# HBioquant/DiffBindFR

Measured on AMD Instinct MI355X. Metric: poses_per_sec, higher is better.
Workload: dtype f32

## Files before the change

### diffbindfr_amd/csrc/conv.hip

```cpp
#include <cstdio>
#include <cstdlib>
#include <type_traits>
#include <vector>

#include "common.h"

#ifndef CONV_PRIO
#define CONV_PRIO 0
#endif
#ifndef CONV_XPF
#define CONV_XPF 0
#endif
#ifndef CONV_NB2_WAVES
#define CONV_NB2_WAVES 2
#endif
#define XS_LD (MAXD + 4)

typedef float f32x4 __attribute__((ext_vector_type(4)));

#define TRACE_BLOCKS 1024
#define TRACE_TILES 48
#define TRACE_REC (2 + 3 * TRACE_TILES + 8)
#define RSTAMP(k) do { if ((ABL & 16) && a.trace && bid < TRACE_BLOCKS && lane == 0) a.trace[((size_t)bid * 4 + wave) * TRACE_REC + 2 + 3 * TRACE_TILES + (k)] = __builtin_amdgcn_s_memrealtime(); } while (0)
#define TSTAMP(k) do { if ((ABL & 16) && a.trace && bid < TRACE_BLOCKS && lane == 0) a.trace[((size_t)bid * 4 + wave) * TRACE_REC + 2 + 3 * TRACE_TILES + (k)] = __builtin_readcyclecounter(); } while (0)
// ... 290 lines not shown
          }
        }
#if CONV_PRIO == 1
        __builtin_amdgcn_s_setprio(0);
#elif CONV_PRIO == 2
        __builtin_amdgcn_s_setprio(3);
#endif
        if ((ABL & 16) && trc && trc_n < TRACE_TILES) {
#pragma unroll
          for (int b = 0; b < NB; ++b) asm volatile("" : "+v"(oacc[b][0]));
          if (lane == 0) trc[4 + 3 * trc_n] = __builtin_readcyclecounter();
          ++trc_n;
        }
      }
      if (flags & 2) {
#pragma unroll
        for (int b = 0; b < NB; ++b) {
          float* op = un + (16 * b + n) * O_LD + oo;
          op[0] = oacc[b][0];
          if (VOUT) { op[1] = oacc[b][1]; op[2] = oacc[b][2]; }
        }
      }
    };
    switch (type) {
      case PT_SS: run(std::integral_constant<int, PT_SS>{}); break;
      case PT_SV: run(std::integral_constant<int, PT_SV>{}); break;
      case PT_VS: run(std::integral_constant<int, PT_VS>{}); break;
      case PT_VVS: run(std::integral_constant<int, PT_VVS>{}); break;
      case PT_VVV: run(std::integral_constant<int, PT_VVV>{}); break;
      default: run(std::integral_constant<int, PT_VTV>{}); break;
    }
  }
  TSTAMP(3);
  RSTAMP(7);
  __syncthreads();
  TSTAMP(4);
  {
    const int d4 = D_out >> 2;
    for (int i = tid; i < ne * d4; i += 256) {
      const int e = i / d4, c4 = i - e * d4;
      *reinterpret_cast<f32x4*>(a.msg + (size_t)(tile0 + e) * D_out + 4 * c4) =
          *reinterpret_cast<const f32x4*>(un + e * O_LD + 4 * c4);
    }
  }
  TSTAMP(5);
}

template <int K, int NB, int ABL>
__global__ __launch_bounds__(256, (NB > 3 ? 1 : NB == 2 ? CONV_NB2_WAVES : 2)) void k_conv(ConvArgs a) {
  conv_body<K, NB, ABL>(a, blockIdx.x);
}

struct ConvLayerArgs { ConvArgs c[4]; int first[5]; };
template <int NB>
__global__ __launch_bounds__(256, (NB > 3 ? 1 : NB == 2 ? CONV_NB2_WAVES : 2)) void k_conv_layer(ConvLayerArgs a) {
  const int b = blockIdx.x;
  const int c = b < a.first[1] ? 0 : b < a.first[2] ? 1 : b < a.first[3] ? 2 : 3;
  conv_body<144, NB, 0>(a.c[c], b - a.first[c]);
}

#ifndef CONV_NB
#define CONV_NB 3
#endif

void launch_conv_layer(const ConvArgs* c4, hipStream_t st) {
  ConvLayerArgs a;
  const int te = 16 * CONV_NB;
  a.first[0] = 0;
  for (int i = 0; i < 4; ++i) { a.c[i] = c4[i]; a.c[i].trace = nullptr; a.first[i + 1] = a.first[i] + (c4[i].max_edges + te - 1) / te; }
  if (a.first[4] <= 0) return;
  hipLaunchKernelGGL((k_conv_layer<CONV_NB>), dim3(a.first[4]), dim3(256), 0, st, a);
}

void launch_conv(const ConvArgs& a, hipStream_t st) {
#ifdef DBFR_DEV_VARIANTS
  static int abl = -1;
  if (abl < 0) { const char* e = getenv("DBFR_CONV_ABL"); abl = e ? atoi(e) : 0; }
#endif
  const int te = 16 * CONV_NB;
  const int tiles = (a.max_edges + te - 1) / te;
  if (tiles <= 0) return;
  ConvArgs b = a;
  b.trace = nullptr;
  static const char* trace_path = getenv("DBFR_CONV_TRACE");
  static int trace_skip = getenv("DBFR_CONV_TRACE_SKIP") ? atoi(getenv("DBFR_CONV_TRACE_SKIP")) : 0;
  if (trace_path && a.w.K == 144 && a.w.W == 7776 && tiles >= 4096 && trace_skip-- <= 0) {
    const size_t nw = (size_t)TRACE_BLOCKS * 4 * TRACE_REC;
    unsigned long long* d = nullptr;
    if (hipMalloc(&d, nw * 8) == hipSuccess) {
      (void)hipMemsetAsync(d, 0, nw * 8, st);
      b.trace = d;
      hipLaunchKernelGGL((k_conv<144, CONV_NB, 16>), dim3(tiles), dim3(256), 0, st, b);
      (void)hipStreamSynchronize(st);
      std::vector<unsigned long long> h(nw);
      (void)hipMemcpy(h.data(), d, nw * 8, hipMemcpyDeviceToHost);
      (void)hipFree(d);
      if (FILE* f = fopen(trace_path, "wb")) { fwrite(h.data(), 8, nw, f); fclose(f); }
      trace_path = nullptr;
      return;
    }
  }
#define LAUNCH(KK, AB) hipLaunchKernelGGL((k_conv<KK, CONV_NB, AB>), dim3(tiles), dim3(256), 0, st, b)
  if (a.w.K != 144) { LAUNCH(96, 0); return; }
#ifdef DBFR_DEV_VARIANTS
  switch (abl) { case 1: LAUNCH(144, 1); return; case 2: LAUNCH(144, 2); return; case 8: LAUNCH(144, 8); return; default: break; }
#endif
  LAUNCH(144, 0);
#undef LAUNCH
}

__device__ __forceinline__ f32x4 row_sum(const float* __restrict__ msg, int rs, int rc, int D, int lane, const uint8_t* __restrict__ first, unsigned long long sc_lanes) {
  const int d4 = D >> 2;
  f32x4 acc = {0.f, 0.f, 0.f, 0.f};
  const f32x4* r = reinterpret_cast<const f32x4*>(msg + (size_t)rs * D) + min(lane, d4 - 1);
  if (!first) {
    if (lane < d4) {
      int e = 0;
      for (; e + 8 <= rc; e += 8) {
        const f32x4 v0 = r[(size_t)e * d4], v1 = r[(size_t)(e + 1) * d4], v2 = r[(size_t)(e + 2) * d4], v3 = r[(size_t)(e + 3) * d4];
        const f32x4 v4 = r[(size_t)(e + 4) * d4], v5 = r[(size_t)(e + 5) * d4], v6 = r[(size_t)(e + 6) * d4], v7 = r[(size_t)(e + 7) * d4];
        acc += v0; acc += v1; acc += v2; acc += v3; acc += v4; acc += v5; acc += v6; acc += v7;
      }
      for (; e + 4 <= rc; e += 4) {
        const f32x4 v0 = r[(size_t)e * d4], v1 = r[(size_t)(e + 1) * d4], v2 = r[(size_t)(e + 2) * d4], v3 = r[(size_t)(e + 3) * d4];
        acc += v0; acc += v1; acc += v2; acc += v3;
      }
      for (; e < rc; ++e) acc += r[(size_t)e * d4];
    }
    return acc;
  }
  const bool sc = (sc_lanes >> lane) & 1ull;
  const f32x4 zero = {0.f, 0.f, 0.f, 0.f};
  for (int e0 = 0; e0 < rc; e0 += 64) {
    const int nb = min(64, rc - e0);
    const unsigned long long fl = __ballot(lane < nb && first[rs + e0 + lane] != 0);
    if (lane < d4) {
      int e = 0;
      auto row = [&](int i) { return (!sc || ((fl >> i) & 1ull)) ? r[(size_t)(e0 + i) * d4] : zero; };
      for (; e + 8 <= nb; e += 8) {
        const f32x4 v0 = row(e), v1 = row(e + 1), v2 = row(e + 2), v3 = row(e + 3), v4 = row(e + 4), v5 = row(e + 5), v6 = row(e + 6), v7 = row(e + 7);
        acc += v0; acc += v1; acc += v2; acc += v3; acc += v4; acc += v5; acc += v6; acc += v7;
      }
      for (; e + 4 <= nb; e += 4) {
        const f32x4 v0 = row(e), v1 = row(e + 1), v2 = row(e + 2), v3 = row(e + 3);
        acc += v0; acc += v1; acc += v2; acc += v3;
      }
      for (; e < nb; ++e)
        if (!sc || ((fl >> e) & 1ull)) acc += r[(size_t)(e0 + e) * d4];
    }
  }
  return acc;
}

__global__ __launch_bounds__(256) void k_reduce_ln(const float* __restrict__ msg, const int* __restrict__ row_start,
                                                   const int* __restrict__ row_cnt, int N, int D, LNDesc ln,
                                                   const float* __restrict__ old, int D_old, float* __restrict__ out,
                                                   int ldo, int mode, const uint8_t* first, unsigned long long sc_lanes) {
  __shared__ float buf[4][MAXD];
  const int lane = threadIdx.x & 63, wave = threadIdx.x >> 6;
  const int node_raw = blockIdx.x * 4 + wave;
  const bool live = node_raw < N;
  const int node = live ? node_raw : N - 1;
  const int rs = row_start[node], rc = row_cnt[node];
  const int d4 = D >> 2;
  const f32x4 acc = row_sum(msg, rs, rc, D, lane, first, sc_lanes);
  if (lane < d4) {
    const float cntf = (float)max(rc, 1);
    float* bw = buf[wave] + 4 * lane;
    bw[0] = acc[0] / cntf; bw[1] = acc[1] / cntf; bw[2] = acc[2] / cntf; bw[3] = acc[3] / cntf;
  }
  __syncthreads();
  int iw = 0, ib = 0;
  for (int bk = 0; bk < ln.nblk; ++bk) {
    const int mul = ln.mul[bk], dim = ln.dim[bk], off = ln.off[bk];
    const int nel = mul * dim;
    float mean[3] = {0.f, 0.f, 0.f};
    for (int i = lane; i < nel; i += 64) {
      int comp = i % dim;
      float v = buf[wave][off + i];
      if (comp == 0) mean[0] += v; else if (comp == 1) mean[1] += v; else mean[2] += v;
    }
#pragma unroll
    for (int c = 0; c < 3; ++c) {
      for (int o = 32; o > 0; o >>= 1) mean[c] += __shfl_xor(mean[c], o);
      mean[c] /= (float)mul;
    }
    float sq = 0.f;
    for (int i = lane; i < nel; i += 64) {
      int u = i / dim, comp = i - u * dim;
      float v = buf[wave][off + i] - (comp == 0 ? mean[0] : comp == 1 ? mean[1] : mean[2]) * ln.mean_shift[iw + u];
      buf[wave][off + i] = v;
      sq += v * v;
    }
    __syncthreads();
    for (int o = 32; o > 0; o >>= 1) sq += __shfl_xor(sq, o);
    const float inv = 1.0f / sqrtf(sq / (float)nel + 1e-5f);
    for (int i = lane; i < nel; i += 64) {
      int u = i / dim;
      float v = buf[wave][off + i] * (inv * ln.weight[iw + u]);
      if (ln.is0e[bk]) v += ln.bias[ib + u];
      buf[wave][off + i] = v;
    }
    iw += mul;
    if (ln.is0e[bk]) ib += mul;
  }
  __syncthreads();
#pragma unroll
  for (int j = 0; j < 3; ++j) {
    int c = lane + 64 * j;
    if (c < D && live) {
      float v = buf[wave][c];
      float* o = out + (size_t)node * ldo + c;
      if (mode == 0) v = (c < D_old ? old[(size_t)node * D_old + c] : 0.f) + v;
      else if (mode == 1) v = *o + v;
      *o = v;
    }
  }
}

void launch_reduce_ln(const float* msg, const int* row_start, const int* row_cnt, int N, int D, const LNDesc& ln,
                      const float* old, int D_old, float* out, int ldo, int mode, hipStream_t st, const uint8_t* first, unsigned long long sc_lanes) {
  if (N <= 0) return;
  hipLaunchKernelGGL(k_reduce_ln, dim3((N + 3) / 4), dim3(256), 0, st, msg, row_start, row_cnt, N, D, ln, old, D_old,
                     out, ldo, mode, first, sc_lanes);
}

struct ReduceLayerArgs {
  const float* msg[4]; const int* row_start[4]; const int* row_cnt[4]; LNDesc ln[4];
  int NL, NA, D, D_old;
  const float* old_l; const float* old_a; float* out_l; float* out_a;
  const uint8_t* first[4]; unsigned long long sc_lanes[4];
};

__device__ __forceinline__ void mean_ln(const float* __restrict__ msg, int rs, int rc, int D, const LNDesc& ln, float* bw, int lane, const uint8_t* first, unsigned long long sc_lanes) {
  const int d4 = D >> 2;
  const f32x4 acc = row_sum(msg, rs, rc, D, lane, first, sc_lanes);
  if (lane < d4) {
    const float cntf = (float)max(rc, 1);
    bw[4 * lane] = acc[0] / cntf; bw[4 * lane + 1] = acc[1] / cntf; bw[4 * lane + 2] = acc[2] / cntf; bw[4 * lane + 3] = acc[3] / cntf;
  }
  __builtin_amdgcn_wave_barrier();
  int iw = 0, ib = 0;
  for (int bk = 0; bk < ln.nblk; ++bk) {
    const int mul = ln.mul[bk], dim = ln.dim[bk], off = ln.off[bk];
    const int nel = mul * dim;
    float mean[3] = {0.f, 0.f, 0.f};
    const bool d3 = dim == 3;
    for (int i = lane; i < nel; i += 64) {
      int comp = d3 ? i % 3 : 0;
      float v = bw[off + i];
      if (comp == 0) mean[0] += v; else if (comp == 1) mean[1] += v; else mean[2] += v;
    }
    for (int o = 32; o > 0; o >>= 1) mean[0] += __shfl_xor(mean[0], o);
    mean[0] /= (float)mul;
    if (d3) {
#pragma unroll
      for (int c = 1; c < 3; ++c) {
        for (int o = 32; o > 0; o >>= 1) mean[c] += __shfl_xor(mean[c], o);
        mean[c] /= (float)mul;
      }
    }
    float sq = 0.f;
    for (int i = lane; i < nel; i += 64) {
      int u = d3 ? i / 3 : i, comp = d3 ? i - 3 * u : 0;
      float v = bw[off + i] - (comp == 0 ? mean[0] : comp == 1 ? mean[1] : mean[2]) * ln.mean_shift[iw + u];
      bw[off + i] = v;
      sq += v * v;
    }
    __builtin_amdgcn_wave_barrier();
    for (int o = 32; o > 0; o >>= 1) sq += __shfl_xor(sq, o);
    const float inv = 1.0f / sqrtf(sq / (float)nel + 1e-5f);
    for (int i = lane; i < nel; i += 64) {
      int u = d3 ? i / 3 : i;
      float v = bw[off + i] * (inv * ln.weight[iw + u]);
      if (ln.is0e[bk]) v += ln.bias[ib + u];
      bw[off + i] = v;
    }
    iw += mul;
    if (ln.is0e[bk]) ib += mul;
  }
  __builtin_amdgcn_wave_barrier();
}

__global__ __launch_bounds__(256) void k_reduce_ln_layer(ReduceLayerArgs a) {
  __shared__ float buf[4][2][MAXD];
  const int lane = threadIdx.x & 63, wave = threadIdx.x >> 6;
  const int nbl = (a.NL + 3) / 4;
  const bool lig = (int)blockIdx.x < nbl;
  const int node = (lig ? blockIdx.x : blockIdx.x - nbl) * 4 + wave;
  const int N = lig ? a.NL : a.NA;
  if (node >= N) return;
  const int s0 = lig ? 0 : 2;
  mean_ln(a.msg[s0], a.row_start[s0][node], a.row_cnt[s0][node], a.D, a.ln[s0], buf[wave][0], lane, a.first[s0], a.sc_lanes[s0]);
  mean_ln(a.msg[s0 + 1], a.row_start[s0 + 1][node], a.row_cnt[s0 + 1][node], a.D, a.ln[s0 + 1], buf[wave][1], lane, a.first[s0 + 1], a.sc_lanes[s0 + 1]);
  const float* old = (lig ? a.old_l : a.old_a) + (size_t)node * a.D_old;
  float* out = (lig ? a.out_l : a.out_a) + (size_t)node * a.D;
#pragma unroll
  for (int j = 0; j < 3; ++j) {
    const int c = lane + 64 * j;
    if (c < a.D) out[c] = ((c < a.D_old ? old[c] : 0.f) + buf[wave][0][c]) + buf[wave][1][c];
  }
}

void launch_reduce_ln_layer(const ReduceLayerArgs& a, hipStream_t st) {
  const int nb = (a.NL + 3) / 4 + (a.NA + 3) / 4;
  if (nb <= 0) return;
  hipLaunchKernelGGL(k_reduce_ln_layer, dim3(nb), dim3(256), 0, st, a);
}
```

### diffbindfr_amd/csrc/graph.hip

```cpp
#include "common.h"

#define MAX_NL 256
#define MAX_NA 8192

enum SetKind { SET_LL = 0, SET_AA = 1, SET_AL = 2, SET_LA = 3, SET_TOR = 4, SET_SC = 5, N_SETS = 6 };

struct GraphArgs {
  dbfr_batch b;
  const int* lig_batch;
  const int* atm_batch;
  const uint8_t* is_cab;
  const int* n_cab;
  const float* tr_sigma;
  float lig_cut2, atom_cut2, cross_cut2;
  int lig_cap, atom_cap, dynamic_cross;
  EdgeSet set[N_SETS];
  int* err;
  int step;
  int lds_nl, lds_na;
  int n_chunk;
  int lanes;
};

__device__ __forceinline__ float d2_rn(float ax, float ay, float az, float bx, float by, float bz) {
// ... 373 lines not shown
    const int t = lane < nl ? tgt[es + lane] : 0;
    unsigned st;
    const int l1 = cut(t, min(32, nl), st);
    if (!f(es, l1, st)) return;
    es += l1;
    if (es >= hi) return;
    const int t2 = __shfl(t, (lane + l1) & 63);
    const int l2 = cut(t2, min(32, hi - es), st);
    if (!f(es, l2, st)) return;
    es += l2;
  }
}
__device__ __forceinline__ void graph_edge_range(const GraphArgs& A, const EdgeSet& S, int g, int& lo, int& hi) {
  const int E = min(*S.n_edges, S.cap);
  lo = min(S.g_base[g * A.n_chunk], E);
  hi = g + 1 < A.b.G ? min(S.g_base[(g + 1) * A.n_chunk], E) : E;
}
__global__ __launch_bounds__(256) void k_chunk_count(GraphArgs A) {
  const EdgeSet& S = A.set[blockIdx.y];
  const int g = blockIdx.x * 4 + (threadIdx.x >> 6);
  if (g >= A.b.G) return;
  int lo = 0, cnt = 0;
  if (S.cap > 0) {
    int hi;
    graph_edge_range(A, S, g, lo, hi);
    chunk_walk(S.tgt, lo, hi, [&](int, int, unsigned) { ++cnt; return true; });
  }
  if ((threadIdx.x & 63) == 0) { S.chunk0[g] = cnt; S.gedge0[g] = lo; }
}
__global__ __launch_bounds__(256) void k_graph_chunks(GraphArgs A) {
  __shared__ int sc[256];
  const EdgeSet& S = A.set[blockIdx.x];
  const int G = A.b.G;
  int running = 0;
  for (int g0 = 0; g0 < G; g0 += 256) {
    const int g = g0 + threadIdx.x;
    const int v = g < G ? S.chunk0[g] : 0;
    sc[threadIdx.x] = v;
    __syncthreads();
    for (int o = 1; o < 256; o <<= 1) {
      const int w = threadIdx.x >= o ? sc[threadIdx.x - o] : 0;
      __syncthreads();
      sc[threadIdx.x] += w;
      __syncthreads();
    }
    if (g < G) S.chunk0[g] = running + sc[threadIdx.x] - v;
    running += sc[255];
    __syncthreads();
  }
  if (threadIdx.x == 0) { S.chunk0[G] = min(running, S.chunk_cap); S.gedge0[G] = S.cap > 0 ? min(*S.n_edges, S.cap) : 0; }
}
__global__ __launch_bounds__(256) void k_chunk_fill(GraphArgs A) {
  const EdgeSet& S = A.set[blockIdx.y];
  const int g = blockIdx.x * 4 + (threadIdx.x >> 6);
  if (g >= A.b.G || S.cap == 0) return;
  int lo, hi;
  graph_edge_range(A, S, g, lo, hi);
  int ch = S.chunk0[g];
  const int lane = threadIdx.x & 63;
  chunk_walk(S.tgt, lo, hi, [&](int es, int len, unsigned starts) {
    if (ch >= S.chunk_cap) return false;
    if (lane == 0) { S.chunk_es[ch] = es; S.chunk_gl[ch] = (g << 6) | len; }
    if (lane < len) S.seg_first[es + lane] = (starts >> lane) & 1u;
    ++ch;
    return true;
  });
}

void launch_graph_chunks(const GraphArgs& A0, hipStream_t st) {
  GraphArgs A = A0;
  if (A.n_chunk <= 0) dbfr_edge_form(A.b, &A.n_chunk, &A.lanes);
  hipLaunchKernelGGL(k_chunk_count, dim3((A.b.G + 3) / 4, N_SETS), dim3(256), 0, st, A);
  hipLaunchKernelGGL(k_graph_chunks, dim3(N_SETS), dim3(256), 0, st, A);
  hipLaunchKernelGGL(k_chunk_fill, dim3((A.b.G + 3) / 4, N_SETS), dim3(256), 0, st, A);
}

__global__ __launch_bounds__(256) void k_flat_chunk_count(const int* tgt, const int* n_edges, int max_edges, int span, int n_span, int* cnt0) {
  const int g = blockIdx.x * 4 + (threadIdx.x >> 6);
  if (g >= n_span) return;
  const int E = min(*n_edges, max_edges);
  const int lo = min(g * span, E), hi = min(lo + span, E);
  int cnt = 0;
  for (int es = lo; es < hi; ++cnt) es += chunk_len(tgt, es, hi);
  if ((threadIdx.x & 63) == 0) cnt0[g] = cnt;
}
__global__ __launch_bounds__(256) void k_flat_chunk_scan(int n_span, int* cnt0, int cap) {
  __shared__ int sc[256];
  int running = 0;
  for (int g0 = 0; g0 < n_span; g0 += 256) {
    const int g = g0 + threadIdx.x;
    const int v = g < n_span ? cnt0[g] : 0;
    sc[threadIdx.x] = v;
    __syncthreads();
    for (int o = 1; o < 256; o <<= 1) {
      const int w = threadIdx.x >= o ? sc[threadIdx.x - o] : 0;
      __syncthreads();
      sc[threadIdx.x] += w;
      __syncthreads();
    }
    if (g < n_span) cnt0[g] = running + sc[threadIdx.x] - v;
    running += sc[255];
    __syncthreads();
  }
  if (threadIdx.x == 0) cnt0[n_span] = min(running, cap);
}
__global__ __launch_bounds__(256) void k_flat_chunk_fill(const int* tgt, const int* n_edges, int max_edges, int span, int n_span, const int* cnt0, int cap,
                                                         int* chunk_es, int* chunk_gl) {
  const int g = blockIdx.x * 4 + (threadIdx.x >> 6);
  if (g >= n_span) return;
  const int E = min(*n_edges, max_edges);
  const int lo = min(g * span, E), hi = min(lo + span, E);
  int ch = cnt0[g];
  for (int es = lo; es < hi && ch < cap; ++ch) {
    const int len = chunk_len(tgt, es, hi);
    if ((threadIdx.x & 63) == 0) { chunk_es[ch] = es; chunk_gl[ch] = len; }
    es += len;
  }
}
void launch_flat_chunks(const int* tgt, const int* n_edges, int max_edges, int span, int n_span, int* cnt0, int cap, int* chunk_es, int* chunk_gl, hipStream_t st) {
  hipLaunchKernelGGL(k_flat_chunk_count, dim3((n_span + 3) / 4), dim3(256), 0, st, tgt, n_edges, max_edges, span, n_span, cnt0);
  hipLaunchKernelGGL(k_flat_chunk_scan, dim3(1), dim3(256), 0, st, n_span, cnt0, cap);
  hipLaunchKernelGGL(k_flat_chunk_fill, dim3((n_span + 3) / 4), dim3(256), 0, st, tgt, n_edges, max_edges, span, n_span, cnt0, cap, chunk_es, chunk_gl);
}

__global__ __launch_bounds__(1024) void k_row_absmax(const float* x0, const int* ptr0, float* out0, const float* x1, const int* ptr1, float* out1, int ld, int D, int G) {
  __shared__ float sm[16];
  const int NT = blockDim.x;
  const bool second = (int)blockIdx.x >= G;
  const int g = second ? blockIdx.x - G : blockIdx.x;
  const float* x = second ? x1 : x0;
  const int* ptr = second ? ptr1 : ptr0;
  const int r0 = ptr[g], r1 = ptr[g + 1];
  const int d4 = D >> 2;
  const long n = (long)(r1 - r0) * d4;
  auto at = [&](long i) {
    const int r = (int)(i / d4), c = (int)(i - (long)r * d4);
    return *reinterpret_cast<const float4*>(x + (size_t)(r0 + r) * ld + 4 * c);
  };
  auto amax = [](float m, const float4& v) { return fmaxf(fmaxf(m, fmaxf(fabsf(v.x), fabsf(v.y))), fmaxf(fabsf(v.z), fabsf(v.w))); };
  float m = 0.f;
  long i = threadIdx.x;
  for (; i + 3 * NT < n; i += 4 * NT) {
    const float4 v0 = at(i), v1 = at(i + NT), v2 = at(i + 2 * NT), v3 = at(i + 3 * NT);
    m = amax(amax(amax(amax(m, v0), v1), v2), v3);
  }
  for (; i < n; i += NT) m = amax(m, at(i));
  for (int o = 1; o < 64; o <<= 1) m = fmaxf(m, __shfl_xor(m, o));
  if ((threadIdx.x & 63) == 0) sm[threadIdx.x >> 6] = m;
  __syncthreads();
  if (threadIdx.x < 16) {
    m = (int)threadIdx.x < (NT >> 6) ? sm[threadIdx.x] : 0.f;
    for (int o = 1; o < 16; o <<= 1) m = fmaxf(m, __shfl_xor(m, o));
    if (threadIdx.x == 0) (second ? out1 : out0)[g] = m;
  }
}
void launch_row_absmax(const float* lx, const int* lig_ptr, float* out_l, const float* ax, const int* atm_ptr, float* out_a, int ld, int D, int G, int n_rows_a, hipStream_t st) {
  if (G <= 0) return;
  const int nt = (long)(n_rows_a / G) * (D >> 2) >= 16384 ? 1024 : 256;
  hipLaunchKernelGGL(k_row_absmax, dim3(2 * G), dim3(nt), 0, st, lx, lig_ptr, out_l, ax, atm_ptr, out_a, ld, D, G);
}

__global__ void k_edge_log(GraphArgs A, int* log, int stride) {
  const int g = blockIdx.x * blockDim.x + threadIdx.x, k = blockIdx.y;
  if (g >= A.b.G) return;
  const EdgeSet& S = A.set[k];
  int c = 0;
  if (S.cap > 0)
    for (int i = 0; i < A.n_chunk; ++i) c += S.g_cnt[g * A.n_chunk + i];
  log[k * stride + g] = c;
}

void launch_edge_log(const GraphArgs& A0, int* log_row, int stride, hipStream_t st) {
  GraphArgs A = A0;
  if (A.n_chunk <= 0) dbfr_edge_form(A.b, &A.n_chunk, &A.lanes);
  hipLaunchKernelGGL(k_edge_log, dim3((A.b.G + 255) / 256, N_SETS), dim3(256), 0, st, A, log_row, stride);
}

__global__ void k_edge_ties(GraphArgs A, int* log, int stride, float tol) {
  const int g = blockIdx.x, k = blockIdx.y;
  const EdgeSet& S = A.set[k];
  __shared__ int total;
  if (threadIdx.x == 0) total = 0;
  __syncthreads();
  int c = 0;
  if (S.cap > 0) {
    const int l0 = A.b.lig_ptr[g], nl = A.b.lig_ptr[g + 1] - l0, a0 = A.b.atm_ptr[g], na = A.b.atm_ptr[g + 1] - a0;
    const float* LP = A.b.lig_pos;
    const float* RP = A.b.rec_pos;
    auto near = [&](float d2, float cut2, float t) {
      const float cut = sqrtf(cut2), e = d2 - cut2;
      return e <= 2.f * cut * t + t * t && (t >= cut || -e <= 2.f * cut * t - t * t);
    };
    if (k == SET_LL || k == SET_AA) {
      const float* P = k == SET_LL ? LP : RP;
      const int p0 = k == SET_LL ? l0 : a0, np = k == SET_LL ? nl : na;
      const float cut2 = k == SET_LL ? A.lig_cut2 : A.atom_cut2;
      for (long idx = threadIdx.x; idx < (long)np * np; idx += blockDim.x) {
        const int i = (int)(idx / np), j = (int)(idx - (long)i * np);
        if (i < j) c += near(d2_rn(P[3 * (p0 + i)], P[3 * (p0 + i) + 1], P[3 * (p0 + i) + 2], P[3 * (p0 + j)], P[3 * (p0 + j) + 1], P[3 * (p0 + j) + 2]), cut2, tol);
      }
    } else if (k == SET_AL || k == SET_LA) {
      const float scale = A.dynamic_cross ? __fadd_rn(__fmul_rn(A.tr_sigma[g], 0.2f), 5.0f) : 1.0f;
      for (long idx = threadIdx.x; idx < (long)nl * na; idx += blockDim.x) {
        const int i = (int)(idx / na), j = (int)(idx - (long)i * na);
        if (A.is_cab[a0 + j]) continue;
        float x0 = LP[3 * (l0 + i)], y0 = LP[3 * (l0 + i) + 1], z0 = LP[3 * (l0 + i) + 2], x1 = RP[3 * (a0 + j)], y1 = RP[3 * (a0 + j) + 1], z1 = RP[3 * (a0 + j) + 2];
        if (A.dynamic_cross) { x0 = __fdiv_rn(x0, scale); y0 = __fdiv_rn(y0, scale); z0 = __fdiv_rn(z0, scale); x1 = __fdiv_rn(x1, scale); y1 = __fdiv_rn(y1, scale); z1 = __fdiv_rn(z1, scale); }
        c += near(d2_rn(x0, y0, z0, x1, y1, z1), A.cross_cut2, tol / scale);
      }
    } else {
      const bool tor = k == SET_TOR;
      const int t0 = tor ? A.b.tor_ptr[g] : A.b.sc_ptr[g], nt = (tor ? A.b.tor_ptr[g + 1] : A.b.sc_ptr[g + 1]) - t0;
      const float* P = tor ? LP : RP;
      const int p0 = tor ? l0 : a0, np = tor ? nl : na;
      const float cut2 = tor ? A.lig_cut2 : A.atom_cut2;
      for (long idx = threadIdx.x; idx < (long)nt * np; idx += blockDim.x) {
        const int t = (int)(idx / np), j = (int)(idx - (long)t * np);
        int u, v;
        if (tor) { const int b = A.b.tor_bond[t0 + t]; u = A.b.bond_src[b]; v = A.b.bond_dst[b]; }
        else { u = A.b.sc_bond[2 * (t0 + t)]; v = A.b.sc_bond[2 * (t0 + t) + 1]; }
        const float mx = (P[3 * u] + P[3 * v]) / 2, my = (P[3 * u + 1] + P[3 * v + 1]) / 2, mz = (P[3 * u + 2] + P[3 * v + 2]) / 2;
        c += near(d2_rn(mx, my, mz, P[3 * (p0 + j)], P[3 * (p0 + j) + 1], P[3 * (p0 + j) + 2]), cut2, tol);
      }
    }
  }
  if (c) atomicAdd(&total, c);
  __syncthreads();
  if (threadIdx.x == 0) log[k * stride + g] = total;
}

void launch_edge_ties(const GraphArgs& A, int* log_row, int stride, float tol, hipStream_t st) {
  hipLaunchKernelGGL(k_edge_ties, dim3(A.b.G, N_SETS), dim3(256), 0, st, A, log_row, stride, tol);
}

__global__ void k_batch_vectors(dbfr_batch b, int* lig_batch, int* atm_batch, uint8_t* is_cab, int* n_cab,
                                int* tor_batch, int* sc_batch) {
  const int g = blockIdx.x;
  for (int i = b.lig_ptr[g] + threadIdx.x; i < b.lig_ptr[g + 1]; i += blockDim.x) lig_batch[i] = g;
  __shared__ int cnt;
  if (threadIdx.x == 0) cnt = 0;
  __syncthreads();
  int c = 0;
  for (int i = b.atm_ptr[g] + threadIdx.x; i < b.atm_ptr[g + 1]; i += blockDim.x) {
    atm_batch[i] = g;
    int a37 = (int)b.pocket_feat[5 * i];
    uint8_t f = (a37 == 1 || a37 == 3);
    is_cab[i] = f;
    c += f;
  }
  atomicAdd(&cnt, c);
  for (int i = b.tor_ptr[g] + threadIdx.x; i < b.tor_ptr[g + 1]; i += blockDim.x) tor_batch[i] = g;
  for (int i = b.sc_ptr[g] + threadIdx.x; i < b.sc_ptr[g + 1]; i += blockDim.x) sc_batch[i] = g;
  __syncthreads();
  if (threadIdx.x == 0) n_cab[g] = cnt;
}

void launch_batch_vectors(const dbfr_batch& b, int* lig_batch, int* atm_batch, uint8_t* is_cab, int* n_cab,
                          int* tor_batch, int* sc_batch, hipStream_t st) {
  hipLaunchKernelGGL(k_batch_vectors, dim3(b.G), dim3(128), 0, st, b, lig_batch, atm_batch, is_cab, n_cab, tor_batch,
                     sc_batch);
}

__global__ void k_time_embed(const float* t, int G, float emb_scale, float* temb) {
  int i = blockIdx.x * blockDim.x + threadIdx.x;
  if (i >= G * EMB) return;
  int g = i / EMB, k = i % EMB;
  const int half = EMB / 2;
  int kk = k % half;
  float neg = -(float)(9.210340371976184 / (half - 1));
  float arg = (float)kk * neg;
  float f = (float)exp((double)arg);
  float x = (emb_scale * t[g]) * f;
  temb[i] = (float)(k < half ? sin((double)x) : cos((double)x));
}

void launch_time_embed(const float* t, int G, float emb_scale, float* temb, hipStream_t st) {
  hipLaunchKernelGGL(k_time_embed, dim3((G * EMB + 255) / 256), dim3(256), 0, st, t, G, emb_scale, temb);
}

enum MlpIn { IN_LIGNODE = 0, IN_LIGEDGE = 1, IN_TG = 2, IN_G = 3 };

struct MlpArgs {
  Mlp2 w;
  int mode;
  const int* n_rows_dev;
  int n_rows_max;
  const float* temb;
  const int* row_graph_tab;
  const int* tgt;
  const int* aux;
  const float* dist;
  const float* bond_feat;
  int nfeat;
  const float* lig_node;
  int nnode;
  const float* gs_offset;
  const float* gs_coeff;
  float* out;
};

#define MLP_ROWS 64
#define MLP_MAXIN 80

__global__ __launch_bounds__(256) void k_mlp(MlpArgs a) {
  __shared__ float xin[MLP_ROWS][MLP_MAXIN + 1];
  __shared__ float hid[MLP_ROWS][NS + 1];
  __shared__ float w0[MLP_MAXIN * NS];
  __shared__ float w1[NS * NS];
  __shared__ float s_gs[EMB];
  const int nrows = a.n_rows_dev ? min(*a.n_rows_dev, a.n_rows_max) : a.n_rows_max;
  if ((int)blockIdx.x * MLP_ROWS >= nrows) return;
  const int in = a.w.in;
  for (int i = threadIdx.x; i < in * NS; i += 256) w0[i] = a.w.w0t[i];
  for (int i = threadIdx.x; i < NS * NS; i += 256) w1[i] = a.w.w1t[i];
  const float coeff = a.gs_coeff ? a.gs_coeff[0] : 0.f;
  if (threadIdx.x < EMB) s_gs[threadIdx.x] = a.gs_offset ? a.gs_offset[threadIdx.x] : 0.f;
  __syncthreads();
  const int kin = (in + 3) & ~3;
  if (kin > in)
    for (int i = threadIdx.x; i < (kin - in) * NS; i += 256) w0[in * NS + i] = 0.f;
  typedef float f32x4 __attribute__((ext_vector_type(4)));
  const int lane = threadIdx.x & 63, wave = threadIdx.x >> 6, n = lane & 15, g = lane >> 4;
  const int row = 16 * wave + n;
  for (int r0 = blockIdx.x * MLP_ROWS; r0 < nrows; r0 += gridDim.x * MLP_ROWS) {
  const int nr = min(MLP_ROWS, nrows - r0);
  {
    const int r = threadIdx.x >> 2, q = threadIdx.x & 3;
    const bool live = r < nr;
    const int arow = r0 + (live ? r : 0);
    const int gph = a.mode == IN_G ? 0 : a.row_graph_tab[a.tgt ? a.tgt[arow] : arow];
    const float dcl = a.dist ? fminf(a.dist[arow], s_gs[EMB - 1]) : 0.f;
    const int bond = a.mode == IN_LIGEDGE ? a.aux[arow] : -1;
    for (int c = q; c < in; c += 4) {
      float v = 0.f;
      if (live) {
        int cc = c;
        if (a.mode == IN_LIGNODE) {
          v = cc < a.nnode ? a.lig_node[(size_t)arow * a.nnode + cc] : a.temb[gph * EMB + cc - a.nnode];
        } else {
          if (a.mode == IN_LIGEDGE) {
            if (cc < a.nfeat) { v = bond >= 0 ? a.bond_feat[(size_t)bond * a.nfeat + cc] : 0.f; cc = -1; }
            else cc -= a.nfeat;
          }
          if (cc >= 0) {
            if (a.mode != IN_G && cc < EMB) v = a.temb[gph * EMB + cc];
            else {
              const int k = a.mode == IN_G ? cc : cc - EMB;
              const float d = dcl - s_gs[k];
              v = expf(coeff * (d * d));
            }
          }
        }
      }
      xin[r][c] = v;
    }
  }
  if (kin > in)
    for (int i = threadIdx.x; i < MLP_ROWS * (kin - in); i += 256) xin[i / (kin - in)][in + i % (kin - in)] = 0.f;
  __syncthreads();
  f32x4 acc[3];
#pragma unroll
  for (int t = 0; t < 3; ++t)
#pragma unroll
    for (int r = 0; r < 4; ++r) acc[t][r] = a.w.b0 ? a.w.b0[16 * t + 4 * g + r] : 0.f;
  for (int k = 0; k < kin; k += 4) {
    const float bv = xin[row][k + g];
#pragma unroll
    for (int t = 0; t < 3; ++t) acc[t] = __builtin_amdgcn_mfma_f32_16x16x4f32(w0[(k + g) * NS + 16 * t + n], bv, acc[t], 0, 0, 0);
  }
#pragma unroll
  for (int t = 0; t < 3; ++t)
#pragma unroll
    for (int r = 0; r < 4; ++r) hid[row][16 * t + 4 * g + r] = fmaxf(acc[t][r], 0.f);
  __syncthreads();
#pragma unroll
  for (int t = 0; t < 3; ++t)
#pragma unroll
    for (int r = 0; r < 4; ++r) acc[t][r] = a.w.b1 ? a.w.b1[16 * t + 4 * g + r] : 0.f;
#pragma unroll
  for (int k = 0; k < NS; k += 4) {
    const float bv = hid[row][k + g];
#pragma unroll
    for (int t = 0; t < 3; ++t) acc[t] = __builtin_amdgcn_mfma_f32_16x16x4f32(w1[(k + g) * NS + 16 * t + n], bv, acc[t], 0, 0, 0);
  }
  if (row < nr) {
#pragma unroll
    for (int t = 0; t < 3; ++t) *reinterpret_cast<f32x4*>(a.out + (size_t)(r0 + row) * NS + 16 * t + 4 * g) = acc[t];
  }
  }
}

void launch_mlp(const MlpArgs& a, hipStream_t st) {
  if (a.n_rows_max <= 0) return;
  const int tiles = (a.n_rows_max + MLP_ROWS - 1) / MLP_ROWS;
  hipLaunchKernelGGL(k_mlp, dim3(tiles < 1024 ? tiles : 1024), dim3(256), 0, st, a);
}

struct AtomEncArgs {
  const float* pocket_feat;
  const int* atm_batch;
  const float* temb;
  const float* emb[5];
  int dims[5];
  const float* lin_t;
  int NA;
  float* out;
};

__global__ __launch_bounds__(256) void k_atom_encoder(AtomEncArgs a) {
  __shared__ float w[(NS + EMB) * NS];
  __shared__ float x[16][NS + EMB];
  for (int i = threadIdx.x; i < (NS + EMB) * NS; i += 256) w[i] = a.lin_t[i];
  const int r0 = blockIdx.x * 16;
  for (int i = threadIdx.x; i < 16 * (NS + EMB); i += 256) {
    int r = i / (NS + EMB), c = i % (NS + EMB);
    int row = r0 + r;
    float v = 0.f;
    if (row < a.NA) {
      if (c < NS) {
        for (int f = 0; f < 5; ++f) {
          int id = (int)a.pocket_feat[(size_t)row * 5 + f];
          id = min(max(id, 0), a.dims[f] - 1);
          v += a.emb[f][(size_t)id * NS + c];
        }
      } else {
        v = a.temb[a.atm_batch[row] * EMB + c - NS];
      }
    }
    x[r][c] = v;
  }
  __syncthreads();
  for (int i = threadIdx.x; i < 16 * NS; i += 256) {
    int r = i / NS, c = i % NS;
    int row = r0 + r;
    if (row >= a.NA) continue;
    float acc = 0.f;
    for (int k = 0; k < NS + EMB; ++k) acc += w[k * NS + c] * x[r][k];
    a.out[(size_t)row * NS + c] = x[r][c] + acc;
  }
}

void launch_atom_encoder(const AtomEncArgs& a, hipStream_t st) {
  if (a.NA <= 0) return;
  hipLaunchKernelGGL(k_atom_encoder, dim3((a.NA + 15) / 16), dim3(256), 0, st, a);
}
```

Baseline: 518.3.

## Specialize reduce-LN and MLP kernels for fixed layouts with register-resident weights

Adds a templated reduce+layer-norm kernel for the known irreps layouts that keeps per-lane values in registers and uses DPP/xor butterflies for the block means and variances. The generic mean_ln path is kept as a fallback. The edge MLP kernel gets templated variants for common input widths that hold the MFMA weight fragments in VGPRs instead of LDS. Because each wave owns its own rows, the block-wide syncthreads are replaced with wave-level barriers, and the next tile's row scalars are prefetched. The trade is higher register pressure and more code paths, for fewer LDS loads and block barriers.

```diff
diff --git a/diffbindfr_amd/csrc/conv.hip b/diffbindfr_amd/csrc/conv.hip
--- a/diffbindfr_amd/csrc/conv.hip
+++ b/diffbindfr_amd/csrc/conv.hip
@@ -616,8 +616,128 @@
   }
 }
 
+template <int O> __device__ __forceinline__ float xor_lane(float x) {
+  if constexpr (O == 8) return __int_as_float(__builtin_amdgcn_update_dpp(0, __float_as_int(x), 0x128, 0xf, 0xf, false));
+  else if constexpr (O == 2) return __int_as_float(__builtin_amdgcn_update_dpp(0, __float_as_int(x), 0x4e, 0xf, 0xf, false));
+  else if constexpr (O == 1) return __int_as_float(__builtin_amdgcn_update_dpp(0, __float_as_int(x), 0xb1, 0xf, 0xf, false));
+  else return __shfl_xor(x, O);
+}
+
+template <int O, int N> __device__ __forceinline__ void xor_stage(float (&x)[N]) {
+  float y[N];
+#pragma unroll
+  for (int i = 0; i < N; ++i) y[i] = xor_lane<O>(x[i]);
+#pragma unroll
+  for (int i = 0; i < N; ++i) x[i] += y[i];
+}
+
+template <int N> __device__ __forceinline__ void xor_butterflies(float (&x)[N]) {
+  xor_stage<32>(x); xor_stage<16>(x); xor_stage<8>(x); xor_stage<4>(x); xor_stage<2>(x); xor_stage<1>(x);
+}
+
+template <int NBLK>
+__global__ __launch_bounds__(256, NBLK == 4 ? 7 : 8) void k_reduce_ln_layer_fixed(ReduceLayerArgs a) {
+  constexpr int D = NBLK == 2 ? 84 : NBLK == 3 ? 120 : MAXD;
+  constexpr int MUL[4] = {48, 12, 12, 48}, DIM[4] = {1, 3, 3, 1}, OFF[4] = {0, 48, 84, 120}, IW[4] = {0, 48, 60, 72};
+  constexpr int NCH = NBLK == 2 ? 4 : NBLK == 3 ? 7 : 8;
+  __shared__ float buf[4][2][MAXD];
+  const int lane = threadIdx.x & 63, wave = threadIdx.x >> 6;
+  const int nbl = (a.NL + 3) / 4;
+  const bool lig = (int)blockIdx.x < nbl;
+  const int node = (lig ? blockIdx.x : blockIdx.x - nbl) * 4 + wave;
+  const int N = lig ? a.NL : a.NA;
+  if (node >= N) return;
+  const int s0 = lig ? 0 : 2;
+  const int rs0 = a.row_start[s0][node], rc0 = a.row_cnt[s0][node], rs1 = a.row_start[s0 + 1][node], rc1 = a.row_cnt[s0 + 1][node];
+  f32x4 acc[2];
+  acc[0] = row_sum(a.msg[s0], rs0, rc0, D, lane, a.first[s0], a.sc_lanes[s0]);
+  acc[1] = row_sum(a.msg[s0 + 1], rs1, rc1, D, lane, a.first[s0 + 1], a.sc_lanes[s0 + 1]);
+  const float* old = (lig ? a.old_l : a.old_a) + (size_t)node * a.D_old;
+  float shift[2][NBLK], weight[2][NBLK], bias[2], oldv[NBLK];
+  unsigned el[NBLK];
+#pragma unroll
+  for (int b = 0; b < NBLK; ++b) {
+    el[b] = min(lane, MUL[b] * DIM[b] - 1);
+    const unsigned un = IW[b] + (DIM[b] == 3 ? el[b] / 3u : el[b]);
+#pragma unroll
+    for (int s = 0; s < 2; ++s) { shift[s][b] = a.ln[s0 + s].mean_shift[un]; weight[s][b] = a.ln[s0 + s].weight[un]; }
+    oldv[b] = OFF[b] + el[b] < (unsigned)a.D_old ? old[OFF[b] + el[b]] : 0.f;
+  }
+#pragma unroll
+  for (int s = 0; s < 2; ++s) bias[s] = a.ln[s0 + s].bias[el[0]];
+  if (lane < D / 4) {
+#pragma unroll
+    for (int s = 0; s < 2; ++s) {
+      const float cntf = (float)max(s ? rc1 : rc0, 1);
+      float* bw = buf[wave][s] + 4 * lane;
+      bw[0] = acc[s][0] / cntf; bw[1] = acc[s][1] / cntf; bw[2] = acc[s][2] / cntf; bw[3] = acc[s][3] / cntf;
+    }
+  }
+  __builtin_amdgcn_wave_barrier();
+  float v[2][NBLK], mean[2 * NCH];
+#pragma unroll
+  for (int s = 0; s < 2; ++s) {
+    int ch = s * NCH;
+#pragma unroll
+    for (int b = 0; b < NBLK; ++b) {
+      v[s][b] = buf[wave][s][OFF[b] + el[b]];
+      const bool in = lane < MUL[b] * DIM[b];
+      const int comp = DIM[b] == 3 ? lane % 3 : 0;
+#pragma unroll
+      for (int c = 0; c < DIM[b]; ++c) mean[ch++] = in && comp == c ? 0.f + v[s][b] : 0.f;
+    }
+  }
+  xor_butterflies(mean);
+  float sq[2 * NBLK];
+#pragma unroll
+  for (int s = 0; s < 2; ++s) {
+    int ch = s * NCH;
+#pragma unroll
+    for (int b = 0; b < NBLK; ++b) {
+      float m[3];
+#pragma unroll
+      for (int c = 0; c < DIM[b]; ++c) m[c] = mean[ch++] / (float)MUL[b];
+      const int comp = DIM[b] == 3 ? lane % 3 : 0;
+      const float mc = DIM[b] == 3 ? (comp == 0 ? m[0] : comp == 1 ? m[1] : m[2]) : m[0];
+      v[s][b] = __builtin_fmaf(-shift[s][b], mc, v[s][b]);
+      sq[s * NBLK + b] = lane < MUL[b] * DIM[b] ? __builtin_fmaf(v[s][b], v[s][b], 0.f) : 0.f;
+    }
+  }
+  xor_butterflies(sq);
+  float* out = (lig ? a.out_l : a.out_a) + (size_t)node * D;
+#pragma unroll
+  for (int b = 0; b < NBLK; ++b) {
+    float r[2];
+#pragma unroll
+    for (int s = 0; s < 2; ++s) {
+      const float inv = 1.0f / sqrtf(sq[s * NBLK + b] / (float)(MUL[b] * DIM[b]) + 1e-5f);
+      r[s] = v[s][b] * (inv * weight[s][b]);
+      asm("" : "+v"(r[s]));
+      if (b == 0) r[s] += bias[s];
+    }
+    if (lane < MUL[b] * DIM[b]) out[OFF[b] + lane] = (oldv[b] + r[0]) + r[1];
+  }
+}
+
+static int reduce_ln_fixed_layout(const ReduceLayerArgs& a) {
+  static const int mul[4] = {48, 12, 12, 48}, dim[4] = {1, 3, 3, 1}, off[4] = {0, 48, 84, 120};
+  const int nblk = a.ln[0].nblk;
+  if (nblk < 2 || nblk > 4 || a.D != off[nblk - 1] + mul[nblk - 1] * dim[nblk - 1] || a.D_old > a.D) return 0;
+  for (int s = 0; s < 4; ++s) {
+    if (a.ln[s].nblk != nblk) return 0;
+    for (int b = 0; b < nblk; ++b)
+      if (a.ln[s].mul[b] != mul[b] || a.ln[s].dim[b] != dim[b] || a.ln[s].off[b] != off[b] || (a.ln[s].is0e[b] != 0) != (b == 0)) return 0;
+  }
+  return nblk;
+}
+
 void launch_reduce_ln_layer(const ReduceLayerArgs& a, hipStream_t st) {
   const int nb = (a.NL + 3) / 4 + (a.NA + 3) / 4;
   if (nb <= 0) return;
-  hipLaunchKernelGGL(k_reduce_ln_layer, dim3(nb), dim3(256), 0, st, a);
-}
+  switch (reduce_ln_fixed_layout(a)) {
+    case 2: hipLaunchKernelGGL(k_reduce_ln_layer_fixed<2>, dim3(nb), dim3(256), 0, st, a); break;
+    case 3: hipLaunchKernelGGL(k_reduce_ln_layer_fixed<3>, dim3(nb), dim3(256), 0, st, a); break;
+    case 4: hipLaunchKernelGGL(k_reduce_ln_layer_fixed<4>, dim3(nb), dim3(256), 0, st, a); break;
+    default: hipLaunchKernelGGL(k_reduce_ln_layer, dim3(nb), dim3(256), 0, st, a);
+  }
+}
diff --git a/diffbindfr_amd/csrc/graph.hip b/diffbindfr_amd/csrc/graph.hip
--- a/diffbindfr_amd/csrc/graph.hip
+++ b/diffbindfr_amd/csrc/graph.hip
@@ -699,35 +699,64 @@
 #define MLP_ROWS 64
 #define MLP_MAXIN 80
 
-__global__ __launch_bounds__(256) void k_mlp(MlpArgs a) {
+__device__ __forceinline__ void wave_lds_order() {
+  __builtin_amdgcn_fence(__ATOMIC_RELEASE, "wavefront");
+  __builtin_amdgcn_wave_barrier();
+  __builtin_amdgcn_fence(__ATOMIC_ACQUIRE, "wavefront");
+}
+
+template <int KS>
+__global__ __launch_bounds__(256, KS == 0 ? 2 : KS > 16 ? 3 : 4) void k_mlp(MlpArgs a) {
   __shared__ float xin[MLP_ROWS][MLP_MAXIN + 1];
   __shared__ float hid[MLP_ROWS][NS + 1];
-  __shared__ float w0[MLP_MAXIN * NS];
-  __shared__ float w1[NS * NS];
+  __shared__ float w0[KS ? 1 : MLP_MAXIN * NS];
+  __shared__ float w1[KS ? 1 : NS * NS];
   __shared__ float s_gs[EMB];
   const int nrows = a.n_rows_dev ? min(*a.n_rows_dev, a.n_rows_max) : a.n_rows_max;
   if ((int)blockIdx.x * MLP_ROWS >= nrows) return;
   const int in = a.w.in;
-  for (int i = threadIdx.x; i < in * NS; i += 256) w0[i] = a.w.w0t[i];
-  for (int i = threadIdx.x; i < NS * NS; i += 256) w1[i] = a.w.w1t[i];
-  const float coeff = a.gs_coeff ? a.gs_coeff[0] : 0.f;
-  if (threadIdx.x < EMB) s_gs[threadIdx.x] = a.gs_offset ? a.gs_offset[threadIdx.x] : 0.f;
-  __syncthreads();
-  const int kin = (in + 3) & ~3;
-  if (kin > in)
-    for (int i = threadIdx.x; i < (kin - in) * NS; i += 256) w0[in * NS + i] = 0.f;
   typedef float f32x4 __attribute__((ext_vector_type(4)));
   const int lane = threadIdx.x & 63, wave = threadIdx.x >> 6, n = lane & 15, g = lane >> 4;
   const int row = 16 * wave + n;
+  const int kin = KS ? 4 * KS : (in + 3) & ~3;
+  float a0[KS ? KS : 1][3], a1[NS / 4][3];
+  if (KS) {
+#pragma unroll
+    for (int ks = 0; ks < KS; ++ks)
+#pragma unroll
+      for (int t = 0; t < 3; ++t) a0[ks][t] = 4 * ks + g < in ? a.w.w0t[(4 * ks + g) * NS + 16 * t + n] : 0.f;
+#pragma unroll
+    for (int ks = 0; ks < NS / 4; ++ks)
+#pragma unroll
+      for (int t = 0; t < 3; ++t) a1[ks][t] = a.w.w1t[(4 * ks + g) * NS + 16 * t + n];
+  } else {
+    for (int i = threadIdx.x; i < in * NS; i += 256) w0[i] = a.w.w0t[i];
+    for (int i = threadIdx.x; i < NS * NS; i += 256) w1[i] = a.w.w1t[i];
+  }
+  const float coeff = a.gs_coeff ? a.gs_coeff[0] : 0.f;
+  if (threadIdx.x < EMB) s_gs[threadIdx.x] = a.gs_offset ? a.gs_offset[threadIdx.x] : 0.f;
+  if (!KS && kin > in)
+    for (int i = threadIdx.x; i < (kin - in) * NS; i += 256) w0[in * NS + i] = 0.f;
+  if (kin > in)
+    for (int i = threadIdx.x; i < MLP_ROWS * (kin - in); i += 256) xin[i / (kin - in)][in + i % (kin - in)] = 0.f;
+  __syncthreads();
+  const int r = threadIdx.x >> 2, q = threadIdx.x & 3;
+  int gph_n = 0, bond_n = -1;
+  float dist_n = 0.f;
+  auto row_scalars = [&](int r0) {
+    const int arow = min(r0 + r, nrows - 1);
+    gph_n = a.mode == IN_G ? 0 : a.row_graph_tab[a.tgt ? a.tgt[arow] : arow];
+    dist_n = a.dist ? a.dist[arow] : 0.f;
+    bond_n = a.mode == IN_LIGEDGE ? a.aux[arow] : -1;
+  };
+  row_scalars(blockIdx.x * MLP_ROWS);
   for (int r0 = blockIdx.x * MLP_ROWS; r0 < nrows; r0 += gridDim.x * MLP_ROWS) {
   const int nr = min(MLP_ROWS, nrows - r0);
   {
-    const int r = threadIdx.x >> 2, q = threadIdx.x & 3;
     const bool live = r < nr;
     const int arow = r0 + (live ? r : 0);
-    const int gph = a.mode == IN_G ? 0 : a.row_graph_tab[a.tgt ? a.tgt[arow] : arow];
-    const float dcl = a.dist ? fminf(a.dist[arow], s_gs[EMB - 1]) : 0.f;
-    const int bond = a.mode == IN_LIGEDGE ? a.aux[arow] : -1;
+    const int gph = gph_n, bond = bond_n;
+    const float dcl = a.dist ? fminf(dist_n, s_gs[EMB - 1]) : 0.f;
     for (int c = q; c < in; c += 4) {
       float v = 0.f;
       if (live) {
@@ -752,24 +781,32 @@
       xin[r][c] = v;
     }
   }
-  if (kin > in)
-    for (int i = threadIdx.x; i < MLP_ROWS * (kin - in); i += 256) xin[i / (kin - in)][in + i % (kin - in)] = 0.f;
-  __syncthreads();
+  wave_lds_order();
+  if (r0 + (int)gridDim.x * MLP_ROWS < nrows) row_scalars(r0 + gridDim.x * MLP_ROWS);
   f32x4 acc[3];
 #pragma unroll
   for (int t = 0; t < 3; ++t)
 #pragma unroll
     for (int r = 0; r < 4; ++r) acc[t][r] = a.w.b0 ? a.w.b0[16 * t + 4 * g + r] : 0.f;
-  for (int k = 0; k < kin; k += 4) {
-    const float bv = xin[row][k + g];
-#pragma unroll
-    for (int t = 0; t < 3; ++t) acc[t] = __builtin_amdgcn_mfma_f32_16x16x4f32(w0[(k + g) * NS + 16 * t + n], bv, acc[t], 0, 0, 0);
+  if (KS) {
+#pragma unroll
+    for (int ks = 0; ks < KS; ++ks) {
+      const float bv = xin[row][4 * ks + g];
+#pragma unroll
+      for (int t = 0; t < 3; ++t) acc[t] = __builtin_amdgcn_mfma_f32_16x16x4f32(a0[ks][t], bv, acc[t], 0, 0, 0);
+    }
+  } else {
+    for (int k = 0; k < kin; k += 4) {
+      const float bv = xin[row][k + g];
+#pragma unroll
+      for (int t = 0; t < 3; ++t) acc[t] = __builtin_amdgcn_mfma_f32_16x16x4f32(w0[(k + g) * NS + 16 * t + n], bv, acc[t], 0, 0, 0);
+    }
   }
 #pragma unroll
   for (int t = 0; t < 3; ++t)
 #pragma unroll
     for (int r = 0; r < 4; ++r) hid[row][16 * t + 4 * g + r] = fmaxf(acc[t][r], 0.f);
-  __syncthreads();
+  wave_lds_order();
 #pragma unroll
   for (int t = 0; t < 3; ++t)
 #pragma unroll
@@ -778,7 +815,7 @@
   for (int k = 0; k < NS; k += 4) {
     const float bv = hid[row][k + g];
 #pragma unroll
-    for (int t = 0; t < 3; ++t) acc[t] = __builtin_amdgcn_mfma_f32_16x16x4f32(w1[(k + g) * NS + 16 * t + n], bv, acc[t], 0, 0, 0);
+    for (int t = 0; t < 3; ++t) acc[t] = __builtin_amdgcn_mfma_f32_16x16x4f32(KS ? a1[k / 4][t] : w1[(k + g) * NS + 16 * t + n], bv, acc[t], 0, 0, 0);
   }
   if (row < nr) {
 #pragma unroll
@@ -790,7 +827,14 @@
 void launch_mlp(const MlpArgs& a, hipStream_t st) {
   if (a.n_rows_max <= 0) return;
   const int tiles = (a.n_rows_max + MLP_ROWS - 1) / MLP_ROWS;
-  hipLaunchKernelGGL(k_mlp, dim3(tiles < 1024 ? tiles : 1024), dim3(256), 0, st, a);
+  const dim3 grid(tiles < 1024 ? tiles : 1024);
+  switch (a.w.hid == NS && a.w.out == NS ? a.w.in : 0) {
+    case 32: hipLaunchKernelGGL(k_mlp<8>, grid, dim3(256), 0, st, a); break;
+    case 59: hipLaunchKernelGGL(k_mlp<15>, grid, dim3(256), 0, st, a); break;
+    case 64: hipLaunchKernelGGL(k_mlp<16>, grid, dim3(256), 0, st, a); break;
+    case 74: hipLaunchKernelGGL(k_mlp<19>, grid, dim3(256), 0, st, a); break;
+    default: hipLaunchKernelGGL(k_mlp<0>, grid, dim3(256), 0, st, a);
+  }
 }
 
 struct AtomEncArgs {
```

New measurement: 533.9, median of 6. +3.0%, better.
